# Iselix/kwiiyatta

Hardware: AMD Instinct MI355X
Metric: frames/sec end-to-end analyse->align->convert->synth, 48 kHz 5 ms hop (higher is better)
Workload: dtype f64; 1 GPU; config3: 48 kHz source (10 s, T=2001) + target (11 s, T=2201) pairs: CheapTrick+D4C of both, pad with freshly drawn silent spectra, sp2mc, FastDTW(radius 32) align, GMM(64 comp, D=144)+MLPG convert, mc2sp, WORLD synthesis; pairs_per_gpu=32, streams_per_gpu=4, GPU_MAX_HW_QUEUES=4, launch=the whole step is one captured HIP graph, gmm_model_prepared=once per converter (the per-mixture matrices depend on the GMM only), parallelism=pairs in lockstep x32 per GPU, pair-per-GPU x1, no collective

## Files before the change

kwiiyatta_amd/csrc/kwy_d4c.hip:

```cpp
#include <math.h>

#include <vector>

#include "kwy_internal.hpp"

#define D4C_FLOOR_F0 47.0
#define D4C_FREQ_INTERVAL 3000.0
#define D4C_MAX_BANDS 8

enum { D4C_HANNING = 1, D4C_BLACKMAN = 2 };

__device__ __forceinline__ double d4c_window(int type, int i, int half, double ratio, int fs, double cf0) {
  const double c1 = kwy_cos_pi_range(KWY_PI * ((2.0 * (i - half) / ratio) / fs) * cf0);
  return type == D4C_HANNING ? 0.5 * c1 + 0.5 : 0.42 + 0.5 * c1 + 0.08 * (2.0 * c1 * c1 - 1.0);
}

struct d4c_window_walk {
  double c, s, cd, sd;
  __device__ __forceinline__ d4c_window_walk(int i0, int step, int half, double ratio, int fs, double cf0) {
    kwy_sincos_pi_range(KWY_PI * ((2.0 * (i0 - half) / ratio) / fs) * cf0, &s, &c);
    sincos(KWY_PI * ((2.0 * step / ratio) / fs) * cf0, &sd, &cd);
  }
  __device__ __forceinline__ void next() { kwy_rotate(c, s, cd, sd); }
  __device__ __forceinline__ double value(int type) const {
// ... 286 lines not shown
      }
      const double w = type == D4C_HANNING ? 0.5 * c1 + 0.5 : 0.42 + 0.5 * c1 + 0.08 * (2.0 * c1 * c1 - 1.0);
      v = __builtin_fma(kwy_randn_from_raw(raw[r]), KWY_SAFE, xv[r] * w);
      Bd[i] = w;
      s1 += v; s2 += w;
    }
    av[r] = v;
  }
  double t1, t2;
  kwy_block_sum2<NT>(s1, s2, red, &t1, &t2);
  const double coef = t1 / t2;
  double pw = 0.0;
#pragma unroll
  for (int r = 0; r < E; ++r) {
    if (tid + NT * r < wl) {
      double v = __builtin_fma(-Bd[tid + NT * r], coef, av[r]);
      av[r] = v;
      pw = __builtin_fma(v, v, pw);
    }
  }
  if (normalise) {
    const double isq = 1.0 / sqrt(kwy_block_sum<NT>(pw, red));
#pragma unroll
    for (int r = 0; r < E; ++r)
      if (tid + NT * r < wl) av[r] = av[r] * isq;
  }
}

template <int NT>
__device__ inline void d4c_subtract_smoothed(double *io, double *S, double *tot, double width, int fs, int N, int kmax) {
  const int H = N / 2;
  int boundary = (int)(width * N / fs) + 1;
  if (boundary > H / 2) boundary = H / 2;
  const int L = min(H + boundary * 2 + 1, kmax + boundary * 2 + 4);
  kwy_block_cumsum_of<NT, D4C_SMOOTH_CHUNK>([&](int i) {
    double m;
    if (i < boundary) m = io[boundary - i];
    else if (i < H + boundary) m = io[i - boundary];
    else m = io[H - (i - (H + boundary))];
    return m * fs / N;
  }, S, L, tot);
  const double origin = -(boundary - 0.5) * fs / N;
  const double inv_dfi = (double)N / fs, inv_width = 1.0 / width;
  const d4c_taps taps = d4c_smoothing_taps(origin, inv_dfi, width);
  for (int k = threadIdx.x; k <= min(H, kmax); k += NT) io[k] = io[k] - d4c_smoothed_bin(S, L, taps, k) * inv_width;
  __syncthreads();
}

template <int NT, int RK>
__device__ inline void d4c_linear_smoothing_regs(const double *in, double (&outv)[RK], double *S, double *tot,
                                                 double width, int fs, int N) {
  const int H = N / 2;
  int boundary = (int)(width * N / fs) + 1;
  if (boundary > H / 2) boundary = H / 2;
  const int L = H + boundary * 2 + 1;
  kwy_block_cumsum_of<NT, D4C_SMOOTH_CHUNK>([&](int i) {
    double m;
    if (i < boundary) m = in[boundary - i];
    else if (i < H + boundary) m = in[i - boundary];
    else m = in[H - (i - (H + boundary))];
    return m * fs / N;
  }, S, L, tot);
  const double origin = -(boundary - 0.5) * fs / N;
  const double inv_dfi = (double)N / fs, inv_width = 1.0 / width;
  const d4c_taps taps = d4c_smoothing_taps(origin, inv_dfi, width);
#pragma unroll
  for (int r = 0; r < RK; ++r) {
    const int k = threadIdx.x + NT * r;
    outv[r] = 0.0;
    if (k <= H) outv[r] = fmax(d4c_smoothed_bin(S, L, taps, k) * inv_width, 0.0);
  }
  __syncthreads();
}

__device__ __forceinline__ kwy_c d4c_opaque(kwy_c v) {
  asm volatile("" : "+v"(v.x), "+v"(v.y));
  return v;
}

template <int LOG2N>
struct d4c_nt { static constexpr int value = LOG2N >= 13 ? 512 : 256; };
template <int LOG2N>
struct d4c_drain { static constexpr bool value = LOG2N == 12; };
#define D4C_DRAIN_TWC(twN, NT, tid) (twN)[((NT) - (tid)) & ((NT) - 1)]
template <int LOG2N>
static constexpr size_t d4c_body_lds() {
  constexpr int N = 1 << LOG2N, H = N / 2, NT = d4c_nt<LOG2N>::value;
  return sizeof(double) * (NT + 16 + D4C_MAX_BANDS + 2) + sizeof(uint32_t) * KWY_EBASE_WORDS +
         (LOG2N >= 12 ? 0 : 8192) + sizeof(double) * ((H + 2) + (2 * H + 2) + 2) +
         ((sizeof(uint32_t) * KWY_SELECT_WORDS(NT) > sizeof(double) * (2 * H + 4))
              ? sizeof(uint32_t) * KWY_SELECT_WORDS(NT) - sizeof(double) * (2 * H + 4) : 0);
}

template <int LOG2N>
__global__ __launch_bounds__(d4c_nt<LOG2N>::value, LOG2N >= 13 ? 1 : 3) void k_d4c_body(
    d4c_batch batch, d4c_params p, kwy_randn_src rs,
    const uint4 *__restrict__ poly, const kwy_c *__restrict__ twH, const kwy_c *__restrict__ twP,
    const kwy_c *__restrict__ twN, long long *__restrict__ dbg) {
  constexpr int N = 1 << LOG2N, H = N / 2;
  constexpr int NT = d4c_nt<LOG2N>::value;
  constexpr int E = N / NT;
  constexpr int RK = (H + 1 + NT - 1) / NT;
  constexpr int HEX = 16 * NT / N;
  static_assert(HEX >= 1, "workgroup narrower than N/16");
  constexpr bool DRAIN = d4c_drain<LOG2N>::value;
#define D4C_STAMP(n) do { if (dbg && threadIdx.x == 0 && blockIdx.x == (unsigned)dbg[63]) dbg[n] = clock64(); } while (0)
  extern __shared__ double smem[];
  double *tot = smem;
  double *red = tot + NT;
  double *coarse = red + 16;
  uint32_t *e = (uint32_t *)(coarse + D4C_MAX_BANDS + 2);
  double *jt_own = (double *)(e + KWY_EBASE_WORDS);
  double *A0 = jt_own + (LOG2N >= 12 ? 0 : 1024);
  kwy_c *B = (kwy_c *)(A0 + (H + 2));
  double *Bd = (double *)B;
  double *P = A0, *Dv = A0;
  double *S = Bd;
  uint4 *jtab = (uint4 *)((LOG2N >= 12) ? A0 : jt_own);

  const int tid = threadIdx.x;
  const int utt = batch.find(blockIdx.x);
  const int64_t frame = (int)blockIdx.x - batch.start[utt];
  const double *__restrict__ x = batch.u[utt].x;
  const int x_length = batch.u[utt].x_length;
  const uint64_t *__restrict__ offs3 = batch.u[utt].offs3;
  const uint64_t *__restrict__ draws_before = batch.u[utt].offs_lt + batch.u[utt].T;
  double *__restrict__ dvbuf = batch.u[utt].dvbuf;
  const double f0v = kwy_uniform(batch.u[utt].f0[frame]);
  double *o = batch.u[utt].out + frame * p.K;
  if (f0v == 0.0 || kwy_uniform(batch.u[utt].ap0[frame]) <= p.threshold) {
    for (int k = tid; k < p.K; k += NT) o[k] = 1.0 - KWY_SAFE;
    return;
  }
  const double cf0 = kwy_uniform(f0v > D4C_FLOOR_F0 ? f0v : D4C_FLOOR_F0);
  const double pos = kwy_uniform(batch.u[utt].tpos[frame]);

  D4C_STAMP(0);
  kwy_c tw4[4];
  kwy_fft_thread_twiddles<LOG2N - 1, NT>(twH, tw4);
#define D4C_BODY_TW4() do { if constexpr (DRAIN) { const int ot = kwy_tid_opaque(); \
    kwy_fft_thread_twiddles<LOG2N - 1, NT>(twH + (ot - (int)threadIdx.x), tw4); } } while (0)
  const kwy_c twb = twN[tid];
  const uint64_t dbase = *draws_before;
  const uint64_t dpos0 = dbase + offs3[3 * frame], dpos1 = dbase + offs3[3 * frame + 1], dpos2 = dbase + offs3[3 * frame + 2];
  const bool cache = dpos2 + (uint64_t)(2 * kwy_matlab_round(4.0 * p.fs / cf0 / 2.0) + 1) <= rs.n;
  const bool zh = 2 * kwy_matlab_round(4.0 * p.fs / cf0 / 2.0) + 1 <= H + 1;

  D4C_STAMP(1);
  constexpr int RP = (H / 2 + NT - 1) / NT;
  double cen_lo[RP], cen_hi[RP];
  double *mid = coarse;
  {
    double av[E];
    for (int which = 0; which < 2; ++which) {
      const int tid = kwy_tid_opaque();
      double cpos = which == 0 ? pos - 0.25 / cf0 : pos + 0.25 / cf0;
      d4c_frame_window<N, NT>(x, x_length, p, cf0, cpos, D4C_BLACKMAN, which == 0 ? dpos0 : dpos1, rs, poly, e, jtab, Bd, true, red, av,
                              A0, cache ? 1 + which : 0);
      __syncthreads();
      if (!(tid & 1)) {
#pragma unroll
        for (int r = 0; r < E; ++r) {
          if (r < E / 2 || !zh || (r == E / 2 && tid == 0)) { const int i = tid + NT * r; Bd[i] = av[r]; Bd[i + 1] = av[r] * (i + 1.0); }
        }
      }
      __syncthreads();
      D4C_STAMP(2 + which * 2);
      D4C_BODY_TW4();
      kwy_fft_inplace_sel_w<LOG2N - 1, NT, false, !DRAIN>(B, tw4, twP, zh);
      kwy_c Ek[RP], Eh[RP];
      if constexpr (DRAIN) {
        static_assert(RP == 4, "four pairs per thread");
        kwy_c Em;
        kwy_fft_tail4_drain<LOG2N - 1, NT, false>(B, Ek, Eh, Em);
        if (tid == 0) { mid[0] = Em.x; mid[1] = Em.y; }
      } else {
#pragma unroll
        for (int r = 0; r < RP; ++r) {
          const int pp = tid + NT * r;
          Ek[r] = Eh[r] = kwy_c{0.0, 0.0};
          if (pp < H / 2) { Ek[r] = B[pp]; Eh[r] = B[(H - pp) & (H - 1)]; }
        }
        if (tid == 0) { mid[0] = B[H / 2].x; mid[1] = B[H / 2].y; }
      }
      __syncthreads();
      if (tid & 1) {
#pragma unroll
        for (int r = 0; r < E; ++r) {
          if (r < E / 2 || !zh) { const int i = tid + NT * r; Bd[i - 1] = av[r]; Bd[i] = av[r] * (i + 1.0); }
        }
      } else if (zh && tid == 0) {
        B[H / 2] = kwy_c{0.0, 0.0};
      }
      __syncthreads();
      D4C_BODY_TW4();
      kwy_fft_inplace_sel_w<LOG2N - 1, NT, false, !DRAIN>(B, tw4, twP, zh);
      kwy_c Od[DRAIN ? 4 : 1], Odh[DRAIN ? 4 : 1], twa = {0.0, 0.0}, twc = {0.0, 0.0};
      if constexpr (DRAIN) {
        kwy_c Om;
        kwy_fft_tail4_drain<LOG2N - 1, NT, false>(B, Od, Odh, Om);
        if (tid == 0) { mid[3] = Om.x; mid[4] = Om.y; }
        twa = twN[tid];
        twc = D4C_DRAIN_TWC(twN, NT, tid);
      }
#pragma unroll
      for (int r = 0; r < RP; ++r) {
        const int pp = tid + NT * r;
        if (DRAIN || pp < H / 2) {
          kwy_c w, Ok, Oh;
          if constexpr (DRAIN) {
            w = kwy_drain_tw<LOG2N - 1, NT>(r, twa, twc);
            Ok = Od[r]; Oh = Odh[r];
          } else {
            w = kwy_tw_hex(d4c_opaque(twb), HEX * r);
            Ok = B[pp]; Oh = B[(H - pp) & (H - 1)];
          }
          const kwy_c t = cmulf(w, Ok);
          const kwy_c u = cmulf(kwy_c{-w.x, w.y}, Oh);
          const kwy_c zp = cadd(Ek[r], t), zhp = csub(Ek[r], t);
          const kwy_c zq = cadd(Eh[r], u), znp = csub(Eh[r], u);
          const double lo = 2.0 * __builtin_fma(zp.x, znp.y, zp.y * znp.x);
          const double hi = 2.0 * __builtin_fma(zq.x, zhp.y, zq.y * zhp.x);
          cen_lo[r] = which == 0 ? lo : cen_lo[r] + lo;
          cen_hi[r] = which == 0 ? hi : cen_hi[r] + hi;
        }
      }
      if (tid == 0) {
        const kwy_c Em = {mid[0], mid[1]}, Om = DRAIN ? kwy_c{mid[3], mid[4]} : B[H / 2];
        const kwy_c t = {Om.y, -Om.x};
        const kwy_c za = cadd(Em, t), zb = csub(Em, t);
        const double v = 2.0 * __builtin_fma(za.x, zb.y, za.y * zb.x);
        mid[2] = which == 0 ? v : mid[2] + v;
      }
      __syncthreads();
      D4C_STAMP(3 + which * 2);
    }

    D4C_STAMP(6);
    d4c_frame_window<N, NT>(x, x_length, p, cf0, pos, D4C_HANNING, dpos2, rs, poly, e, jtab, Bd, false, red, av, A0, cache ? 2 : 0);
#pragma unroll
    for (int r = 0; r < E; ++r)
      if (r < E / 2 || !zh) Bd[tid + NT * r] = av[r];
    if (zh && tid == 0) { Bd[H] = av[E / 2]; Bd[H + 1] = 0.0; }
    __syncthreads();
  }
  D4C_STAMP(7);
  D4C_BODY_TW4();
  kwy_fft_inplace_sel_w<LOG2N - 1, NT, false, !DRAIN>(B, tw4, twP, zh);
  D4C_STAMP(8);
  double pv[RK];
  if constexpr (DRAIN) {
    static_assert(RK == 9, "four pairs per thread and the self-paired bin");
    const int tid = kwy_tid_opaque();
    kwy_c lo[4], hi[4], md;
    kwy_fft_tail4_drain<LOG2N - 1, NT, false>(B, lo, hi, md);
    const kwy_c twa = twN[tid], twc = D4C_DRAIN_TWC(twN, NT, tid);
#pragma unroll
    for (int s = 0; s < 4; ++s) {
      if (s == 0 && tid == 0) kwy_rfft_pair_power2_dc(lo[0], &pv[0], &pv[1]);
      else kwy_rfft_pair_power2_v(lo[s], hi[s], kwy_drain_tw<LOG2N - 1, NT>(s, twa, twc), &pv[2 * s], &pv[2 * s + 1]);
    }
    pv[8] = 0.0;
    if (tid == 0) {
      double pm;
      kwy_rfft_pair_power2_v(md, md, kwy_c{0.0, -1.0}, &pv[8], &pm);
    }
    __syncthreads();
#pragma unroll
    for (int s = 0; s < 4; ++s) {
      const int k = kwy_drain_bin<LOG2N - 1>(s, tid);
      P[k] = pv[2 * s];
      P[H - k] = pv[2 * s + 1];
    }
    if (tid == 0) P[H / 2] = pv[8];
  } else {
    constexpr int Q = (H / 2) / NT;
    static_assert(RK == 2 * Q + 1, "pairs per thread");
#pragma unroll
    for (int q = 0; q < Q; ++q)
      kwy_rfft_pair_power2_w<LOG2N - 1>(B, tid + NT * q, kwy_tw_hex(d4c_opaque(twb), HEX * q), &pv[2 * q], &pv[2 * q + 1]);
    pv[2 * Q] = 0.0;
    if (tid == 0) {
      double pm;
      kwy_rfft_pair_power2_w<LOG2N - 1>(B, H / 2, kwy_c{0.0, -1.0}, &pv[2 * Q], &pm);
    }
    __syncthreads();
#pragma unroll
    for (int q = 0; q < Q; ++q) {
      const int k = tid + NT * q;
      P[k] = pv[2 * q];
      P[H - k] = pv[2 * q + 1];
    }
    if (tid == 0) P[H / 2] = pv[2 * Q];
  }
  __syncthreads();
  d4c_dc_correction<NT>(P, S, cf0, p.fs, N);
  d4c_linear_smoothing_regs<NT, RK>(P, pv, S, tot, cf0, p.fs, N);

  D4C_STAMP(9);
#pragma unroll
  for (int r = 0; r < RP; ++r) {
    const int pp = DRAIN ? kwy_drain_bin<LOG2N - 1>(r, tid) : tid + NT * r;
    if (pp < H / 2) { Dv[pp] = cen_lo[r]; Dv[H - pp] = cen_hi[r]; }
  }
  if (tid == 0) Dv[H / 2] = mid[2];
  __syncthreads();
  d4c_dc_correction<NT>(Dv, S, cf0, p.fs, N);
#pragma unroll
  for (int r = 0; r < RK; ++r)
    if (tid + NT * r <= H) Dv[tid + NT * r] = Dv[tid + NT * r] / pv[r];
  __syncthreads();
  const int kdv = p.dv_len - 1;
  d4c_linear_smoothing<NT>(Dv, Dv, S, tot, cf0 / 2.0, p.fs, N, kdv + 2 * ((int)(cf0 * N / p.fs) + 1) + 4);
  d4c_subtract_smoothed<NT>(Dv, S, tot, cf0, p.fs, N, kdv);

  D4C_STAMP(10);
  {
    double *dv = dvbuf + (size_t)frame * p.dv_stride;
    for (int k = tid; k < p.dv_len; k += NT) dv[k] = Dv[k];
  }
  D4C_STAMP(15);
#undef D4C_STAMP
#undef D4C_BODY_TW4
}

template <int LOG2N>
static constexpr size_t d4c_bands_lds() {
  constexpr int N = 1 << LOG2N, H = N / 2, NT = d4c_nt<LOG2N>::value;
  constexpr size_t sel = sizeof(uint32_t) * (KWY_SELECT_WORDS(NT) + (d4c_drain<LOG2N>::value ? 0 : KWY_SELECT_WIDE_WORDS));
  return sizeof(double) * (16 + D4C_MAX_BANDS + 2 + 2 * NT) + sizeof(double) * ((2 * H + 2) + 2) +
         (sel > sizeof(double) * (2 * H + 4) ? sel - sizeof(double) * (2 * H + 4) : 0);
}

template <int LOG2N, bool SPARSE>
__global__ __launch_bounds__(d4c_nt<LOG2N>::value, LOG2N >= 13 ? 2 : 4) void k_d4c_bands(
    d4c_batch batch, d4c_params p, const kwy_c *__restrict__ twH, const kwy_c *__restrict__ twP,
    const kwy_c *__restrict__ twN, const double *__restrict__ nuttall, long long *__restrict__ dbg) {
  constexpr int N = 1 << LOG2N, H = N / 2;
// ... 368 lines not shown
```

kwiiyatta_amd/csrc/kwy_device.hpp:

```cpp
#pragma once

#include <hip/hip_runtime.h>
#include <stdint.h>

#define KWY_THREADS 256
#define KWY_WAVES (KWY_THREADS / 64)
#define KWY_PI 3.1415926535897932384
#define KWY_SAFE 0.000000000001
#define KWY_DBL_MAX 1.79769313486231570815e+308
static_assert(1.0 - KWY_SAFE == 1.0 - 1e-12, "the two spellings of the safe guard are one double");

struct kwy_rng {
  uint32_t x, y, z, w;
};

__device__ __forceinline__ void kwy_rng_seed(kwy_rng &r) {
  r.x = 123456789u; r.y = 362436069u; r.z = 521288629u; r.w = 88675123u;
}

__device__ __forceinline__ uint32_t kwy_rng_step(kwy_rng &r) {
  uint32_t t = r.x ^ (r.x << 11);
  r.x = r.y; r.y = r.z; r.z = r.w;
  r.w = (r.w ^ (r.w >> 19)) ^ (t ^ (t >> 8));
  return r.w;
// ... 1278 lines not shown
      const double er = 0.5 * (A.x + Bc.x);
      const double dr = 0.5 * (A.x - Bc.x), di = 0.5 * (A.y + Bc.y);
      const double orr = di, oi = -dr;
      const double pr = __builtin_fma(orr, w.x, -(oi * w.y));
      double a = er + pr, b = er - pr;
      a *= 2.0;
      b *= 2.0;
      lo[r] = a;
      hi[r] = b;
    }
  }
  __syncthreads();
#pragma unroll
  for (int r = 0; r < R; ++r) {
    const int k = tid + NT * r;
    if (k > H / 2) continue;
    L[k] = lo[r];
    if (k != H - k) L[H - k] = hi[r];
  }
  if constexpr (ZEROS) {
    for (int n = H + 1 + tid; n < N; n += NT) L[n] = 0.0;
  }
  __syncthreads();
}

template <int LOG2H>
__device__ __forceinline__ kwy_c kwy_rfft_bin_w(const kwy_c *z, int k, kwy_c w) {
  constexpr int H = 1 << LOG2H;
  if (k == 0) return {z[0].x + z[0].y, 0.0};
  if (k == H) return {z[0].x - z[0].y, 0.0};
  const kwy_c A = z[k];
  const kwy_c B = {z[H - k].x, -z[H - k].y};
  const double er = 0.5 * (A.x + B.x), ei = 0.5 * (A.y + B.y);
  const double dr = 0.5 * (A.x - B.x), di = 0.5 * (A.y - B.y);
  const double orr = di, oi = -dr;
  return {er + (orr * w.x - oi * w.y), ei + (orr * w.y + oi * w.x)};
}
template <int LOG2H>
__device__ __forceinline__ kwy_c kwy_rfft_bin2_w(const kwy_c *z, int k, kwy_c w) {
  constexpr int H = 1 << LOG2H;
  if (k == 0) return {2.0 * (z[0].x + z[0].y), 0.0};
  if (k == H) return {2.0 * (z[0].x - z[0].y), 0.0};
  const kwy_c A = z[k];
  const kwy_c B = {z[H - k].x, -z[H - k].y};
  const double er = A.x + B.x, ei = A.y + B.y;
  const double dr = A.x - B.x, di = A.y - B.y;
  return {__builtin_fma(dr, w.y, __builtin_fma(di, w.x, er)), __builtin_fma(-dr, w.x, __builtin_fma(di, w.y, ei))};
}
template <int LOG2H>
__device__ __forceinline__ void kwy_rfft_pair_power2_w(const kwy_c *z, int k, kwy_c w, double *pk, double *pm) {
  constexpr int H = 1 << LOG2H;
  if (k == 0) {
    const double a = 2.0 * (z[0].x + z[0].y), b = 2.0 * (z[0].x - z[0].y);
    *pk = a * a; *pm = b * b;
    return;
  }
  const kwy_c A = z[k], Bz = z[H - k];
  const double er = A.x + Bz.x, ei = A.y - Bz.y;
  const double dr = A.x - Bz.x, di = A.y + Bz.y;
  const double pr = __builtin_fma(dr, w.y, di * w.x), pi = __builtin_fma(-dr, w.x, di * w.y);
  const double xr = er + pr, xi = ei + pi, yr = er - pr, yi = ei - pi;
  *pk = __builtin_fma(xr, xr, xi * xi);
  *pm = __builtin_fma(yr, yr, yi * yi);
}
__device__ __forceinline__ kwy_c kwy_rfft_bin2_v(kwy_c A, kwy_c Bz, kwy_c w) {
  const kwy_c B = {Bz.x, -Bz.y};
  const double er = A.x + B.x, ei = A.y + B.y;
  const double dr = A.x - B.x, di = A.y - B.y;
  return {__builtin_fma(dr, w.y, __builtin_fma(di, w.x, er)), __builtin_fma(-dr, w.x, __builtin_fma(di, w.y, ei))};
}
__device__ __forceinline__ void kwy_rfft_pair_power2_v(kwy_c A, kwy_c Bz, kwy_c w, double *pk, double *pm) {
  const double er = A.x + Bz.x, ei = A.y - Bz.y;
  const double dr = A.x - Bz.x, di = A.y + Bz.y;
  const double pr = __builtin_fma(dr, w.y, di * w.x), pi = __builtin_fma(-dr, w.x, di * w.y);
  const double xr = er + pr, xi = ei + pi, yr = er - pr, yi = ei - pi;
  *pk = __builtin_fma(xr, xr, xi * xi);
  *pm = __builtin_fma(yr, yr, yi * yi);
}
__device__ __forceinline__ void kwy_rfft_pair_power2_dc(kwy_c Z0, double *pk, double *pm) {
  const double a = 2.0 * (Z0.x + Z0.y), b = 2.0 * (Z0.x - Z0.y);
  *pk = a * a; *pm = b * b;
}

template <int LOG2H, int NT, bool INV>
__device__ __forceinline__ void kwy_fft_tail4_drain(const kwy_c *z, kwy_c (&lo)[4], kwy_c (&hi)[4], kwy_c &mid) {
  constexpr int H = 1 << LOG2H, Q = H / 4;
  static_assert(LOG2H % 3 == 2 && NT == Q / 2, "radix-4 tail, two butterflies per thread");
  const int t = kwy_tid_opaque();
  const int jb = t ? Q - t : Q / 2;
  kwy_c a[4], b[4];
#pragma unroll
  for (int m = 0; m < 4; ++m) { a[m] = z[t + m * Q]; b[m] = z[jb + m * Q]; }
  {
    const kwy_c apc = cadd(a[0], a[2]), amc = csub(a[0], a[2]);
    const kwy_c bpd = cadd(a[1], a[3]), jq = kwy_rot90<INV>(csub(a[1], a[3]));
    a[0] = cadd(apc, bpd); a[1] = cadd(amc, jq); a[2] = csub(apc, bpd); a[3] = csub(amc, jq);
  }
  {
    const kwy_c apc = cadd(b[0], b[2]), amc = csub(b[0], b[2]);
    const kwy_c bpd = cadd(b[1], b[3]), jq = kwy_rot90<INV>(csub(b[1], b[3]));
    b[0] = cadd(apc, bpd); b[1] = cadd(amc, jq); b[2] = csub(apc, bpd); b[3] = csub(amc, jq);
  }
  const bool t0 = t == 0;
  lo[0] = a[0]; hi[0] = t0 ? a[0] : b[3];
  lo[1] = a[1]; hi[1] = t0 ? a[3] : b[2];
  lo[2] = b[0]; hi[2] = t0 ? b[3] : a[3];
  lo[3] = b[1]; hi[3] = t0 ? b[2] : a[2];
  mid = a[2];
}
template <int LOG2H>
__device__ __forceinline__ int kwy_drain_bin(int s, int t) {
  constexpr int Q = (1 << LOG2H) / 4;
  switch (s) {
    case 0: return t;
    case 1: return Q + t;
    case 2: return t ? Q - t : Q / 2;
    default: return t ? 2 * Q - t : Q + Q / 2;
  }
}
template <int LOG2H, int NT>
__device__ __forceinline__ kwy_c kwy_drain_tw(int s, kwy_c twa, kwy_c twc) {
  constexpr int HEX = 16 * NT / (2 << LOG2H);
  static_assert(HEX >= 1, "workgroup narrower than N/16");
  switch (s) {
    case 0: return kwy_tw_hex(twa, 0);
    case 1: return kwy_tw_hex(twa, 2 * HEX);
    case 2: return kwy_tw_hex(twc, HEX);
    default: return kwy_tw_hex(twc, 3 * HEX);
  }
}

template <int LOG2H>
__device__ __forceinline__ kwy_c kwy_rfft_bin(const kwy_c *z, int k, const kwy_c *__restrict__ twN) {
  return kwy_rfft_bin_w<LOG2H>(z, k, twN[k & ((2 << LOG2H) - 1)]);
}

__device__ __forceinline__ int kwy_matlab_round(double x) {
  return x > 0 ? (int)(x + 0.5) : (int)(x - 0.5);
}
```

kwiiyatta_amd/csrc/kwy_selftest.h:

```cpp
#ifndef KWY_SELFTEST_H_
#define KWY_SELFTEST_H_
#ifdef __cplusplus
extern "C" {
#endif
int kwy_debug_smallest_sum_dev(void *stream, const double *values, int problems, int n, int m, double *out);
int kwy_debug_select_paths_dev(void *stream, const double *values, int problems, int n, int m, double *out_ref,
                               double *out_new);
int kwy_debug_select_paths512_dev(void *stream, const double *values, int problems, int n, int m, double *out_ref,
                                  double *out_new);
int kwy_debug_devmath_dev(void *stream, const double *x, int n, double *log_out, double *sin_out, double *cos_out);
int kwy_debug_block_exscan_dev(void *stream, const int *values, int problems, int *offsets, int *totals);
int kwy_debug_rfft_paths_dev(void *stream, const double *x, int problems, int log2n, double *out_old, double *out_new);
int kwy_debug_fft_powers_dev(void *stream, const double *x, int problems, int log2h, int nt, int inverse,
                             double *out_lane, double *out_table, double *tab, double *tab_ref, double *tab_ref_conj);
int kwy_debug_syn_first_passes_dev(void *stream, const double *x, int problems, double *out_dense, double *out_sparse,
                                   double *out_half, double *fold_ref, double *fold_new);
int kwy_debug_fft_half_w_dev(void *stream, const double *x, const double *stale, int problems, int log2h, int inverse,
                             int tail, double *out_dense, double *out_half);
#ifdef __cplusplus
}
#endif
#endif
```

kwiiyatta_amd/csrc/selftest/kwy_selftest.hip:

```cpp
#include <hip/hip_runtime.h>

#include <math.h>
#include <stdint.h>

#include <vector>

#include "../kwy_device.hpp"
#include "../kwy_selftest.h"

#define D4C_NT 256

__global__ __launch_bounds__(D4C_NT) void k_select_selftest(const double *__restrict__ v, int n, int m,
                                                           double *__restrict__ out) {
  constexpr int RK = 9;
  __shared__ __attribute__((aligned(16))) uint32_t hist[KWY_SELECT_WORDS(D4C_NT) + KWY_SELECT_WIDE_WORDS];
  __shared__ double red[2 * D4C_NT / 64];
  const int tid = threadIdx.x;
  const double *x = v + (size_t)blockIdx.x * n;
  unsigned long long key[RK];
#pragma unroll
  for (int r = 0; r < RK; ++r) {
    const int k = tid + D4C_NT * r;
    key[r] = k < n ? (unsigned long long)__double_as_longlong(x[k]) : ~0ull;
  }
// ... 455 lines not shown
  if (rc == 0) {
    const size_t lds = sizeof(kwy_c) * (H + 1);
    hipLaunchKernelGGL(k_twiddle_powers_fill<0>, dim3(1), dim3(64), 0, s, (const kwy_c *)tw, tw + H / 8 + N,
                       KWY_TWP_ENTRIES(LOG2H));
    hipLaunchKernelGGL(k_syn_first_passes_selftest<0>, dim3(problems), dim3(128), lds, s, (const kwy_c *)x, (const kwy_c *)tw,
                       (const kwy_c *)(tw + H / 8 + N), (const kwy_c *)(tw + H / 8), (kwy_c *)out_dense, (kwy_c *)out_sparse,
                       (kwy_c *)out_half, fold_ref, fold_new);
    if (hipGetLastError() != hipSuccess) rc = -2;
  }
  if (hipStreamSynchronize(s) != hipSuccess) rc = -2;
  (void)hipFree(tw);
  return rc;
}

template <int LOG2H, int NT, bool INV, bool TAIL>
__global__ __launch_bounds__(NT) void k_fft_half_w_selftest(const kwy_c *__restrict__ x, const kwy_c *__restrict__ stale,
                                                            const kwy_c *__restrict__ twH, const kwy_c *__restrict__ twP,
                                                            kwy_c *__restrict__ out_dense, kwy_c *__restrict__ out_half) {
  constexpr int H = 1 << LOG2H;
  extern __shared__ double smem[];
  kwy_c *B = (kwy_c *)smem;
  const int tid = threadIdx.x;
  const kwy_c *row = x + (size_t)blockIdx.x * H, *old = stale + (size_t)blockIdx.x * H;
  kwy_c tw4[4];
  kwy_fft_thread_twiddles<LOG2H, NT>(twH, tw4);
#pragma nounroll
  for (int path = 0; path < 2; ++path) {
    kwy_c *o = (path == 0 ? out_dense : out_half) + (size_t)blockIdx.x * H;
    for (int i = tid; i < H; i += NT) B[i] = (path == 0 || i <= H / 2) ? row[i] : old[i];
    __syncthreads();
    if (path == 0) kwy_fft_inplace_w<LOG2H, NT, INV, TAIL>(B, tw4, twP);
    else kwy_fft_inplace_half_w<LOG2H, NT, INV, TAIL>(B, tw4, twP);
    for (int i = tid; i < H; i += NT) o[i] = B[i];
    __syncthreads();
  }
}

template <int LOG2H, int NT, bool INV, bool TAIL>
static int fft_half_w_launch(hipStream_t stream, const kwy_c *x, const kwy_c *stale, int problems, const kwy_c *twH,
                             const kwy_c *twP, kwy_c *out_dense, kwy_c *out_half) {
  const size_t lds = sizeof(kwy_c) * (1 << LOG2H);
  auto kern = k_fft_half_w_selftest<LOG2H, NT, INV, TAIL>;
  if (hipFuncSetAttribute((const void *)kern, hipFuncAttributeMaxDynamicSharedMemorySize, (int)lds) != hipSuccess) return -2;
  hipLaunchKernelGGL(kern, dim3(problems), dim3(NT), lds, stream, x, stale, twH, twP, out_dense, out_half);
  return hipGetLastError() == hipSuccess ? 0 : -2;
}
template <int LOG2H, int NT>
static int fft_half_w_pick(hipStream_t s, bool inv, bool tail, const kwy_c *x, const kwy_c *stale, int problems,
                           const kwy_c *twH, const kwy_c *twP, kwy_c *od, kwy_c *oh) {
  if (inv) return tail ? fft_half_w_launch<LOG2H, NT, true, true>(s, x, stale, problems, twH, twP, od, oh)
                       : fft_half_w_launch<LOG2H, NT, true, false>(s, x, stale, problems, twH, twP, od, oh);
  return tail ? fft_half_w_launch<LOG2H, NT, false, true>(s, x, stale, problems, twH, twP, od, oh)
              : fft_half_w_launch<LOG2H, NT, false, false>(s, x, stale, problems, twH, twP, od, oh);
}

extern "C" int kwy_debug_fft_half_w_dev(void *stream, const double *x, const double *stale, int problems, int log2h,
                                        int inverse, int tail, double *out_dense, double *out_half) {
  if (!x || !stale || !out_dense || !out_half || problems <= 0) return -1;
  if (log2h < 10 || log2h > 12) return -1;
  const int H = 1 << log2h, entries = H / 512;
  std::vector<kwy_c> h(H / 8);
  for (int k = 0; k < H / 8; ++k) { const double a = -2.0 * M_PI * (double)k / (double)H; h[k] = {cos(a), sin(a)}; }
  kwy_c *tw = nullptr;
  if (hipMalloc((void **)&tw, sizeof(kwy_c) * (H / 8 + KWY_TWP_ENTRY * entries)) != hipSuccess) return -2;
  int rc = 0;
  hipStream_t s = (hipStream_t)stream;
  if (hipMemcpy(tw, h.data(), sizeof(kwy_c) * (H / 8), hipMemcpyHostToDevice) != hipSuccess) rc = -2;
  if (rc == 0) {
    kwy_c *tp = tw + H / 8;
    hipLaunchKernelGGL(k_twiddle_powers_fill<0>, dim3(1), dim3(64), 0, s, (const kwy_c *)tw, tp, entries);
    if (hipGetLastError() != hipSuccess) rc = -2;
    const kwy_c *cx = (const kwy_c *)x, *cs = (const kwy_c *)stale;
    kwy_c *od = (kwy_c *)out_dense, *oh = (kwy_c *)out_half;
    if (rc == 0) {
      if (log2h == 10) rc = fft_half_w_pick<10, 256>(s, inverse != 0, tail != 0, cx, cs, problems, tw, tp, od, oh);
      else if (log2h == 11) rc = fft_half_w_pick<11, 256>(s, inverse != 0, tail != 0, cx, cs, problems, tw, tp, od, oh);
      else rc = fft_half_w_pick<12, 512>(s, inverse != 0, tail != 0, cx, cs, problems, tw, tp, od, oh);
    }
  }
  if (hipStreamSynchronize(s) != hipSuccess) rc = -2;
  (void)hipFree(tw);
  return rc;
}
```

Baseline: 3.041 million frames/s.

## Use wave-local FFT passes in the D4C body for the 4096-point transform

For the LOG2N==12 D4C body kernel, the half-size complex FFT now runs a first pass that writes a swizzled LDS layout. The remaining passes are arranged so each wavefront touches only its own data, and a wave-level lgkmcnt fence replaces a workgroup barrier between them. A matching drain reads the final pairs back from that layout. This removes __syncthreads barriers and aims for conflict-free LDS access, at the cost of a hard-coded H=2048/NT=256 layout whose correctness rests on the wave-ownership assumption; a selftest comparing the old and new paths is added.

```diff
diff --git a/kwiiyatta_amd/csrc/kwy_d4c.hip b/kwiiyatta_amd/csrc/kwy_d4c.hip
--- a/kwiiyatta_amd/csrc/kwy_d4c.hip
+++ b/kwiiyatta_amd/csrc/kwy_d4c.hip
@@ -392,6 +392,23 @@
 struct d4c_nt { static constexpr int value = LOG2N >= 13 ? 512 : 256; };
 template <int LOG2N>
 struct d4c_drain { static constexpr bool value = LOG2N == 12; };
+template <int LOG2N>
+struct d4c_body_wl { static constexpr bool value = LOG2N == 12; };
+template <int LOG2H, int NT, bool WL>
+__device__ __forceinline__ void d4c_thread_twiddles(const kwy_c *__restrict__ twH, int t, kwy_c (&w)[4]) {
+  if constexpr (WL) kwy_fftwl_thread_twiddles(twH, t, w);
+  else kwy_fft_thread_twiddles<LOG2H, NT>(twH + (t - (int)threadIdx.x), w);
+}
+template <int LOG2H, int NT, bool WL>
+__device__ __forceinline__ void d4c_fft_sel(kwy_c *z, const kwy_c (&w)[4], const kwy_c *__restrict__ pw, bool half) {
+  if constexpr (WL) { kwy_fftwl_first_sel<false>(z, kwy_tw_reg{w[0]}, half); kwy_fftwl_rest<false>(z, kwy_tw_reg{w[1]}, pw); }
+  else kwy_fft_inplace_sel_w<LOG2H, NT, false, false>(z, w, pw, half);
+}
+template <int LOG2H, int NT, bool WL>
+__device__ __forceinline__ void d4c_fft_drain(const kwy_c *z, kwy_c (&lo)[4], kwy_c (&hi)[4], kwy_c &mid) {
+  if constexpr (WL) kwy_fftwl_tail4_drain<false>(z, lo, hi, mid);
+  else kwy_fft_tail4_drain<LOG2H, NT, false>(z, lo, hi, mid);
+}
 #define D4C_DRAIN_TWC(twN, NT, tid) (twN)[((NT) - (tid)) & ((NT) - 1)]
 template <int LOG2N>
 static constexpr size_t d4c_body_lds() {
@@ -414,6 +431,8 @@
   constexpr int HEX = 16 * NT / N;
   static_assert(HEX >= 1, "workgroup narrower than N/16");
   constexpr bool DRAIN = d4c_drain<LOG2N>::value;
+  constexpr bool WL = d4c_body_wl<LOG2N>::value;
+  static_assert(!WL || DRAIN, "the wave-local transform ends in the drained pass");
 #define D4C_STAMP(n) do { if (dbg && threadIdx.x == 0 && blockIdx.x == (unsigned)dbg[63]) dbg[n] = clock64(); } while (0)
   extern __shared__ double smem[];
   double *tot = smem;
@@ -449,7 +468,7 @@
   kwy_c tw4[4];
   kwy_fft_thread_twiddles<LOG2N - 1, NT>(twH, tw4);
 #define D4C_BODY_TW4() do { if constexpr (DRAIN) { const int ot = kwy_tid_opaque(); \
-    kwy_fft_thread_twiddles<LOG2N - 1, NT>(twH + (ot - (int)threadIdx.x), tw4); } } while (0)
+    d4c_thread_twiddles<LOG2N - 1, NT, WL>(twH, ot, tw4); } } while (0)
   const kwy_c twb = twN[tid];
   const uint64_t dbase = *draws_before;
   const uint64_t dpos0 = dbase + offs3[3 * frame], dpos1 = dbase + offs3[3 * frame + 1], dpos2 = dbase + offs3[3 * frame + 2];
@@ -477,12 +496,13 @@
       __syncthreads();
       D4C_STAMP(2 + which * 2);
       D4C_BODY_TW4();
-      kwy_fft_inplace_sel_w<LOG2N - 1, NT, false, !DRAIN>(B, tw4, twP, zh);
+      if constexpr (DRAIN) d4c_fft_sel<LOG2N - 1, NT, WL>(B, tw4, twP, zh);
+      else kwy_fft_inplace_sel_w<LOG2N - 1, NT, false, true>(B, tw4, twP, zh);
       kwy_c Ek[RP], Eh[RP];
       if constexpr (DRAIN) {
         static_assert(RP == 4, "four pairs per thread");
         kwy_c Em;
-        kwy_fft_tail4_drain<LOG2N - 1, NT, false>(B, Ek, Eh, Em);
+        d4c_fft_drain<LOG2N - 1, NT, WL>(B, Ek, Eh, Em);
         if (tid == 0) { mid[0] = Em.x; mid[1] = Em.y; }
       } else {
 #pragma unroll
@@ -504,11 +524,12 @@
       }
       __syncthreads();
       D4C_BODY_TW4();
-      kwy_fft_inplace_sel_w<LOG2N - 1, NT, false, !DRAIN>(B, tw4, twP, zh);
+      if constexpr (DRAIN) d4c_fft_sel<LOG2N - 1, NT, WL>(B, tw4, twP, zh);
+      else kwy_fft_inplace_sel_w<LOG2N - 1, NT, false, true>(B, tw4, twP, zh);
       kwy_c Od[DRAIN ? 4 : 1], Odh[DRAIN ? 4 : 1], twa = {0.0, 0.0}, twc = {0.0, 0.0};
       if constexpr (DRAIN) {
         kwy_c Om;
-        kwy_fft_tail4_drain<LOG2N - 1, NT, false>(B, Od, Odh, Om);
+        d4c_fft_drain<LOG2N - 1, NT, WL>(B, Od, Odh, Om);
         if (tid == 0) { mid[3] = Om.x; mid[4] = Om.y; }
         twa = twN[tid];
         twc = D4C_DRAIN_TWC(twN, NT, tid);
@@ -556,14 +577,15 @@
   }
   D4C_STAMP(7);
   D4C_BODY_TW4();
-  kwy_fft_inplace_sel_w<LOG2N - 1, NT, false, !DRAIN>(B, tw4, twP, zh);
+  if constexpr (DRAIN) d4c_fft_sel<LOG2N - 1, NT, WL>(B, tw4, twP, zh);
+  else kwy_fft_inplace_sel_w<LOG2N - 1, NT, false, true>(B, tw4, twP, zh);
   D4C_STAMP(8);
   double pv[RK];
   if constexpr (DRAIN) {
     static_assert(RK == 9, "four pairs per thread and the self-paired bin");
     const int tid = kwy_tid_opaque();
     kwy_c lo[4], hi[4], md;
-    kwy_fft_tail4_drain<LOG2N - 1, NT, false>(B, lo, hi, md);
+    d4c_fft_drain<LOG2N - 1, NT, WL>(B, lo, hi, md);
     const kwy_c twa = twN[tid], twc = D4C_DRAIN_TWC(twN, NT, tid);
 #pragma unroll
     for (int s = 0; s < 4; ++s) {
diff --git a/kwiiyatta_amd/csrc/kwy_device.hpp b/kwiiyatta_amd/csrc/kwy_device.hpp
--- a/kwiiyatta_amd/csrc/kwy_device.hpp
+++ b/kwiiyatta_amd/csrc/kwy_device.hpp
@@ -1384,6 +1384,25 @@
   *pk = a * a; *pm = b * b;
 }
 
+template <bool INV>
+__device__ __forceinline__ void kwy_tail4_drain_pairs(kwy_c (&a)[4], kwy_c (&b)[4], bool t0, kwy_c (&lo)[4],
+                                                      kwy_c (&hi)[4], kwy_c &mid) {
+  {
+    const kwy_c apc = cadd(a[0], a[2]), amc = csub(a[0], a[2]);
+    const kwy_c bpd = cadd(a[1], a[3]), jq = kwy_rot90<INV>(csub(a[1], a[3]));
+    a[0] = cadd(apc, bpd); a[1] = cadd(amc, jq); a[2] = csub(apc, bpd); a[3] = csub(amc, jq);
+  }
+  {
+    const kwy_c apc = cadd(b[0], b[2]), amc = csub(b[0], b[2]);
+    const kwy_c bpd = cadd(b[1], b[3]), jq = kwy_rot90<INV>(csub(b[1], b[3]));
+    b[0] = cadd(apc, bpd); b[1] = cadd(amc, jq); b[2] = csub(apc, bpd); b[3] = csub(amc, jq);
+  }
+  lo[0] = a[0]; hi[0] = t0 ? a[0] : b[3];
+  lo[1] = a[1]; hi[1] = t0 ? a[3] : b[2];
+  lo[2] = b[0]; hi[2] = t0 ? b[3] : a[3];
+  lo[3] = b[1]; hi[3] = t0 ? b[2] : a[2];
+  mid = a[2];
+}
 template <int LOG2H, int NT, bool INV>
 __device__ __forceinline__ void kwy_fft_tail4_drain(const kwy_c *z, kwy_c (&lo)[4], kwy_c (&hi)[4], kwy_c &mid) {
   constexpr int H = 1 << LOG2H, Q = H / 4;
@@ -1393,22 +1412,7 @@
   kwy_c a[4], b[4];
 #pragma unroll
   for (int m = 0; m < 4; ++m) { a[m] = z[t + m * Q]; b[m] = z[jb + m * Q]; }
-  {
-    const kwy_c apc = cadd(a[0], a[2]), amc = csub(a[0], a[2]);
-    const kwy_c bpd = cadd(a[1], a[3]), jq = kwy_rot90<INV>(csub(a[1], a[3]));
-    a[0] = cadd(apc, bpd); a[1] = cadd(amc, jq); a[2] = csub(apc, bpd); a[3] = csub(amc, jq);
-  }
-  {
-    const kwy_c apc = cadd(b[0], b[2]), amc = csub(b[0], b[2]);
-    const kwy_c bpd = cadd(b[1], b[3]), jq = kwy_rot90<INV>(csub(b[1], b[3]));
-    b[0] = cadd(apc, bpd); b[1] = cadd(amc, jq); b[2] = csub(apc, bpd); b[3] = csub(amc, jq);
-  }
-  const bool t0 = t == 0;
-  lo[0] = a[0]; hi[0] = t0 ? a[0] : b[3];
-  lo[1] = a[1]; hi[1] = t0 ? a[3] : b[2];
-  lo[2] = b[0]; hi[2] = t0 ? b[3] : a[3];
-  lo[3] = b[1]; hi[3] = t0 ? b[2] : a[2];
-  mid = a[2];
+  kwy_tail4_drain_pairs<INV>(a, b, t == 0, lo, hi, mid);
 }
 template <int LOG2H>
 __device__ __forceinline__ int kwy_drain_bin(int s, int t) {
@@ -1432,6 +1436,124 @@
   }
 }
 
+__device__ __forceinline__ void kwy_lds_wave_fence() {
+  asm volatile("s_waitcnt lgkmcnt(0)" ::: "memory");
+}
+__device__ __forceinline__ void kwy_fftwl_thread_twiddles(const kwy_c *__restrict__ twH, int t, kwy_c (&w)[4]) {
+  w[0] = twH[t];
+  w[1] = twH[32 * ((t >> 3) & 7) + 8 * ((t >> 6) & 3)];
+  w[2] = w[3] = kwy_c{1.0, 0.0};
+}
+__device__ __forceinline__ void kwy_fftwl_store_first(kwy_c *z, int j, const kwy_c (&a)[8]) {
+  const int c = j ^ (((j >> 5) & 1) << 3);
+#pragma unroll
+  for (int m = 0; m < 8; ++m) z[256 * m + (c ^ (m ^ ((m & 4) << 1)))] = a[m];
+}
+template <bool INV>
+__device__ __forceinline__ void kwy_fftwl_twiddle(kwy_c (&a)[8], kwy_c w1) {
+  if (INV) w1.y = -w1.y;
+  const kwy_c w2 = cmulf(w1, w1), w4 = cmulf(w2, w2);
+  const kwy_c w3 = cmulf(w1, w2), w5 = cmulf(w4, w1), w6 = cmulf(w4, w2);
+  const kwy_c w7 = cmulf(w4, w3);
+  a[1] = cmulf(w1, a[1]); a[2] = cmulf(w2, a[2]); a[3] = cmulf(w3, a[3]);
+  a[4] = cmulf(w4, a[4]); a[5] = cmulf(w5, a[5]); a[6] = cmulf(w6, a[6]);
+  a[7] = cmulf(w7, a[7]);
+}
+template <bool INV>
+__device__ __forceinline__ void kwy_fftwl_first_sel(kwy_c *z, kwy_tw_reg tw, bool half) {
+  constexpr int H = 2048, Q = 256;
+  const int j = kwy_tid_opaque();
+  kwy_c a[8];
+#pragma unroll
+  for (int m = 0; m < 4; ++m) a[m] = z[j + m * Q];
+  if (half) {
+    a[4] = {0.0, 0.0};
+    if (j == 0) a[4] = z[H / 2];
+    kwy_dft8_low5<INV>(a);
+  } else {
+#pragma unroll
+    for (int m = 4; m < 8; ++m) a[m] = z[j + m * Q];
+    kwy_dft8<INV>(a);
+  }
+  kwy_fftwl_twiddle<INV>(a, tw(j));
+  kwy_fftwl_store_first(z, j, a);
+  __syncthreads();
+}
+template <bool INV>
+__device__ __forceinline__ void kwy_fftwl_first_sparse(kwy_c *z, kwy_tw_reg tw, kwy_c a0, kwy_c a1) {
+  const int j = kwy_tid_opaque();
+  kwy_c a[8];
+  if (j == 0) {
+    a[0] = a0; a[1] = a1;
+#pragma unroll
+    for (int m = 2; m < 8; ++m) a[m] = {0.0, 0.0};
+    kwy_dft8<INV>(a);
+  } else {
+    kwy_c w1 = tw(j);
+    if (INV) w1.y = -w1.y;
+    const kwy_c w2 = cmulf(w1, w1), w4 = cmulf(w2, w2);
+    const kwy_c w3 = cmulf(w1, w2), w5 = cmulf(w4, w1), w6 = cmulf(w4, w2);
+    const kwy_c w7 = cmulf(w4, w3);
+    a[0] = a0; a[1] = cmulf(w1, a0); a[2] = cmulf(w2, a0); a[3] = cmulf(w3, a0);
+    a[4] = cmulf(w4, a0); a[5] = cmulf(w5, a0); a[6] = cmulf(w6, a0); a[7] = cmulf(w7, a0);
+  }
+  kwy_fftwl_store_first(z, j, a);
+  __syncthreads();
+}
+template <bool INV>
+__device__ __forceinline__ void kwy_fftwl_rest(kwy_c *z, kwy_tw_reg tw1, const kwy_c *__restrict__ pw) {
+  const int t = kwy_tid_opaque();
+  const int s = t & 7, hi3 = (t >> 3) & 7, wv = (t >> 6) & 3;
+  const int sw = s ^ ((s & 4) << 1);
+  kwy_c a[8];
+  {
+    const int c = 256 * s + ((4 * hi3 + wv) ^ sw);
+    const int at[2] = {c, c ^ 8};
+#pragma unroll
+    for (int m = 0; m < 8; ++m) a[m] = z[at[m & 1] + 32 * m];
+    kwy_dft8<INV>(a);
+    kwy_fftwl_twiddle<INV>(a, tw1(0));
+#pragma unroll
+    for (int m = 0; m < 8; ++m) z[at[m & 1] + 32 * m] = a[m];
+  }
+  kwy_lds_wave_fence();
+  {
+    const int k = sw ^ ((hi3 & 1) << 3);
+    const int c = 256 * s + 32 * hi3 + (wv ^ (k & 3));
+    int at[4];
+#pragma unroll
+    for (int q = 0; q < 4; ++q) at[q] = c + 4 * (q ^ (k >> 2));
+#pragma unroll
+    for (int m = 0; m < 8; ++m) a[m] = z[at[m & 3] + 4 * (m & 4)];
+    kwy_dft8<INV>(a);
+    const kwy_c *__restrict__ pe = pw + KWY_TWP_ENTRY * __builtin_amdgcn_readfirstlane(t >> 6);
+#pragma unroll
+    for (int m = 1; m < 8; ++m) {
+      kwy_c w = pe[m];
+      if (INV) w.y = -w.y;
+      a[m] = cmulf(w, a[m]);
+    }
+#pragma unroll
+    for (int m = 0; m < 8; ++m) z[at[m & 3] + 4 * (m & 4)] = a[m];
+  }
+  __syncthreads();
+}
+__device__ __forceinline__ int kwy_fftwl_tail_at(int j, int j2) {
+  const int s = j & 7, m1 = (j >> 3) & 7, m2 = (j >> 6) & 7;
+  const int k = s ^ ((s & 4) << 1) ^ ((m1 & 1) << 3);
+  return 256 * s + 32 * m1 + ((4 * m2) ^ (k & 12)) + (j2 ^ (k & 3));
+}
+template <bool INV>
+__device__ __forceinline__ void kwy_fftwl_tail4_drain(const kwy_c *z, kwy_c (&lo)[4], kwy_c (&hi)[4], kwy_c &mid) {
+  constexpr int Q = 512;
+  const int t = kwy_tid_opaque();
+  const int jb = t ? Q - t : Q / 2;
+  kwy_c a[4], b[4];
+#pragma unroll
+  for (int m = 0; m < 4; ++m) { a[m] = z[kwy_fftwl_tail_at(t, m)]; b[m] = z[kwy_fftwl_tail_at(jb, m)]; }
+  kwy_tail4_drain_pairs<INV>(a, b, t == 0, lo, hi, mid);
+}
+
 template <int LOG2H>
 __device__ __forceinline__ kwy_c kwy_rfft_bin(const kwy_c *z, int k, const kwy_c *__restrict__ twN) {
   return kwy_rfft_bin_w<LOG2H>(z, k, twN[k & ((2 << LOG2H) - 1)]);
diff --git a/kwiiyatta_amd/csrc/kwy_selftest.h b/kwiiyatta_amd/csrc/kwy_selftest.h
--- a/kwiiyatta_amd/csrc/kwy_selftest.h
+++ b/kwiiyatta_amd/csrc/kwy_selftest.h
@@ -17,6 +17,8 @@
                                    double *out_half, double *fold_ref, double *fold_new);
 int kwy_debug_fft_half_w_dev(void *stream, const double *x, const double *stale, int problems, int log2h, int inverse,
                              int tail, double *out_dense, double *out_half);
+int kwy_debug_fft_wave_local_dev(void *stream, const double *x, const double *stale, int problems, int kind,
+                                 double *out_old, double *out_new);
 #ifdef __cplusplus
 }
 #endif
diff --git a/kwiiyatta_amd/csrc/selftest/kwy_selftest.hip b/kwiiyatta_amd/csrc/selftest/kwy_selftest.hip
--- a/kwiiyatta_amd/csrc/selftest/kwy_selftest.hip
+++ b/kwiiyatta_amd/csrc/selftest/kwy_selftest.hip
@@ -561,3 +561,77 @@
   (void)hipFree(tw);
   return rc;
 }
+
+template <bool SPARSE>
+__global__ __launch_bounds__(256) void k_fft_wave_local_selftest(const kwy_c *__restrict__ x, const kwy_c *__restrict__ stale,
+                                                                 const kwy_c *__restrict__ twH, const kwy_c *__restrict__ twP,
+                                                                 int kind, kwy_c *__restrict__ out_old,
+                                                                 kwy_c *__restrict__ out_new) {
+  constexpr int LOG2H = 11, H = 1 << LOG2H, NT = 256;
+  extern __shared__ double smem[];
+  kwy_c *B = (kwy_c *)smem;
+  const int tid = threadIdx.x;
+  const kwy_c *row = x + (size_t)blockIdx.x * H, *old = stale + (size_t)blockIdx.x * (H + 1);
+  const bool half = kind == 1 || kind == 2;
+#pragma nounroll
+  for (int path = 0; path < 2; ++path) {
+    kwy_c *o = (path == 0 ? out_old : out_new) + ((size_t)blockIdx.x * NT + tid) * 9;
+    for (int i = tid; i <= H; i += NT) B[i] = old[i];
+    __syncthreads();
+    if (!SPARSE) {
+      const int n = half ? H / 2 + 1 : H;
+      for (int i = tid; i < n; i += NT) B[i] = (kind == 2 && i == H / 2) ? kwy_c{0.0, 0.0} : row[i];
+      __syncthreads();
+    }
+    kwy_c tw4[4], lo[4], hi[4], md;
+    if (path == 0) {
+      kwy_fft_thread_twiddles<LOG2H, NT>(twH, tw4);
+      if constexpr (SPARSE) {
+        kwy_fft_pass8_first_sparse_core<LOG2H, NT, false>(B, kwy_tw_reg{tw4[0]}, row[tid], tid == 0 ? row[H / 8] : kwy_c{0.0, 0.0});
+        kwy_fft_inplace_rest_w<LOG2H, NT, false, false>(B, tw4, twP);
+      } else {
+        kwy_fft_inplace_sel_w<LOG2H, NT, false, false>(B, tw4, twP, half);
+      }
+      kwy_fft_tail4_drain<LOG2H, NT, false>(B, lo, hi, md);
+    } else {
+      kwy_fftwl_thread_twiddles(twH, tid, tw4);
+      if constexpr (SPARSE) kwy_fftwl_first_sparse<false>(B, kwy_tw_reg{tw4[0]}, row[tid], tid == 0 ? row[H / 8] : kwy_c{0.0, 0.0});
+      else kwy_fftwl_first_sel<false>(B, kwy_tw_reg{tw4[0]}, half);
+      kwy_fftwl_rest<false>(B, kwy_tw_reg{tw4[1]}, twP);
+      kwy_fftwl_tail4_drain<false>(B, lo, hi, md);
+    }
+#pragma unroll
+    for (int s = 0; s < 4; ++s) { o[s] = lo[s]; o[4 + s] = hi[s]; }
+    o[8] = md;
+    __syncthreads();
+  }
+}
+
+extern "C" int kwy_debug_fft_wave_local_dev(void *stream, const double *x, const double *stale, int problems, int kind,
+                                            double *out_old, double *out_new) {
+  if (!x || !stale || !out_old || !out_new || problems <= 0 || kind < 0 || kind > 3) return -1;
+  constexpr int LOG2H = 11, H = 1 << LOG2H, entries = KWY_TWP_ENTRIES(LOG2H);
+  std::vector<kwy_c> h(H / 8);
+  for (int k = 0; k < H / 8; ++k) { const double a = -2.0 * M_PI * (double)k / (double)H; h[k] = {cos(a), sin(a)}; }
+  kwy_c *tw = nullptr;
+  if (hipMalloc((void **)&tw, sizeof(kwy_c) * (H / 8 + KWY_TWP_ENTRY * entries)) != hipSuccess) return -2;
+  int rc = 0;
+  hipStream_t s = (hipStream_t)stream;
+  if (hipMemcpy(tw, h.data(), sizeof(kwy_c) * (H / 8), hipMemcpyHostToDevice) != hipSuccess) rc = -2;
+  if (rc == 0) {
+    kwy_c *tp = tw + H / 8;
+    hipLaunchKernelGGL(k_twiddle_powers_fill<0>, dim3(1), dim3(64), 0, s, (const kwy_c *)tw, tp, entries);
+    if (hipGetLastError() != hipSuccess) rc = -2;
+    const size_t lds = sizeof(kwy_c) * (H + 1);
+    auto kern = kind == 3 ? k_fft_wave_local_selftest<true> : k_fft_wave_local_selftest<false>;
+    if (rc == 0 && hipFuncSetAttribute((const void *)kern, hipFuncAttributeMaxDynamicSharedMemorySize, (int)lds) != hipSuccess) rc = -2;
+    if (rc == 0) {
+      hipLaunchKernelGGL(kern, dim3(problems), dim3(256), lds, s, (const kwy_c *)x, (const kwy_c *)stale, (const kwy_c *)tw,
+                         (const kwy_c *)tp, kind, (kwy_c *)out_old, (kwy_c *)out_new);
+      if (hipGetLastError() != hipSuccess) rc = -2;
+    }
+  }
+  if (hipStreamSynchronize(s) != hipSuccess) rc = -2;
+  (void)hipFree(tw);
+  return rc;
+}
```

After: 3.072 million frames/s, median of 6. 1.01x the previous value.
